# Frikallo/parakeet.cpp

Hardware: AMD Instinct MI355X
Metric: RTFx (audio-sec/wall-sec), mel+encoder+TDT decode, tdt-ctc-110m 10s@b64 (higher is better)
Workload: dtype f32; 1 GPU; tdt-ctc-110m, batch=64x10s clips per GPU, TDT greedy decode (the loops of 4 consecutive steps driven as one lock-step batch), fp32 (BASELINE configs[1]); parallelism=dp1 (utterance shards, no data-path collective), decode_group=4, decode_loop=phases, decode_overlap=1

## Files before the change

parakeet.cpp_amd/csrc/kernels/attention.hip:

```cpp
#include "attention_dev.hpp"

namespace pk {

#ifndef ATT_OCC
#define ATT_OCC 4
#endif

template <int HD, int VCH, bool SG = false, bool RAG = false, int OCC = (HD <= 64 ? ATT_OCC : 2), bool BAND = false>
__global__ __launch_bounds__(256, OCC) void relpos_attention_kernel(const float *__restrict__ qkv, int ldq, int d, int T,
                                                               const float *__restrict__ pos ,
                                                               const float *__restrict__ bias_u, const float *__restrict__ bias_v,
                                                               float scale, float *__restrict__ ctx, int PITS, int n_rb, int n_bh,
                                                               float *__restrict__ s_scratch, int ctx_bf16, int pos_row0, SeqRag rg, int left, int right) {
    static_assert(!(BAND && SG), "the band form keeps its score block in LDS");
    __builtin_amdgcn_s_setprio(3);
    constexpr int NQ4 = HD / 16;
    constexpr int VPIT = HD + 16;
    constexpr int NDV = HD / 32;
    extern __shared__ __attribute__((aligned(16))) float smem[];
    const int SPLANE = att_score_plane(PITS);
    const AttScores sc{SG ? s_scratch + (size_t)blockIdx.x * 4 * SPLANE : smem, SPLANE, PITS};
    float *VS = SG ? smem : smem + 4 * SPLANE;
    const int H = d / HD;
    AttPlace pl;
    if (!att_place<RAG, RB>(H, T, n_rb, n_bh, rg, pl)) return;
    const int h = pl.h, i0 = pl.i0;
    const int64_t row0 = pl.row0;
    T = pl.T;
    if constexpr (RAG && !BAND) pos_row0 = rg.pos_T - T;
    const int rows = (T - i0) < RB ? (T - i0) : RB;
    const AttWave w = att_wave();
    int jlo = 0, jhi = T - 1;
    if constexpr (BAND) {
        jlo = i0 - left > 0 ? i0 - left : 0;
        jhi = i0 + RB - 1 + right < T - 1 ? i0 + RB - 1 + right : T - 1;
    }
    const int W = BAND ? jhi - jlo + 1 : T;
    const int NP = BAND ? left + right + 1 : 2 * T - 1;
    const bool has_pos = BAND || pos != nullptr;
    const float *qb = qkv + row0 * ldq + h * HD;
    const float *kb = qb + d + (int64_t)jlo * ldq, *vb = qb + 2 * d + (int64_t)jlo * ldq;
    const float *pb = pos + (BAND ? (int64_t)0 : (int64_t)pos_row0 * d) + h * HD;

    float4 qx[NQ4];
    ATT_STAMP(4, 0);
    att_load_q_biased(qb, ldq, i0 + w.rt * 16, T, bias_u, h * HD, has_pos, w.l15, w.kq, qx);
    ATT_STAMP(4, 1);
    att_content_pass(sc, w, kb, ldq, W, qx, has_pos, scale);
    ATT_STAMP(4, 2);
    if (has_pos) att_load_q_biased(qb, ldq, i0 + w.rt * 16, T, bias_v, h * HD, true, w.l15, w.kq, qx);
    const int w_lo = i0 + w.rt * 16, w_hi = (w_lo + 15) < (T - 1) ? (w_lo + 15) : (T - 1);
    int wpmin = T - 1 - w_hi, wpmax = 2 * T - 2 - w_lo;
    if constexpr (BAND) {
        wpmin = jlo - w_hi + left > 0 ? jlo - w_hi + left : 0;
        wpmax = jhi - w_lo + left < NP - 1 ? jhi - w_lo + left : NP - 1;
    }
    const int npt = (has_pos && w_lo < T) ? (wpmax - wpmin) / 16 + 1 : 0;
    att_shift_pass(sc, w, pb, d, NP, wpmin, npt, BAND ? left + jlo : T - 1, i0, T, W, qx, scale);
    ATT_STAMP(4, 4);
    float4 vf[VCH * (HD / 4) / 256];
    att_v_issue<HD, VCH, 256>(vb, ldq, 0, W, vf);
    __syncthreads();
    ATT_STAMP(4, 5);
    if constexpr (BAND) {
        AttRowsBand band;
#pragma unroll
        for (int k = 0; k < RB / 4; ++k) {
            const int i = i0 + w.wave + 4 * k;
            band.clo[k] = (i - left > jlo ? i - left : jlo) - jlo;
            band.chi[k] = i < T ? (i + right < jhi ? i + right : jhi) - jlo : -1;
        }
        att_softmax(sc, w, W, ctx_bf16, band);
    } else {
        att_softmax(sc, w, W, ctx_bf16, AttRowsFull{});
    }
    ATT_STAMP(4, 6);
    att_v_commit<HD, VCH, 256>(VS, vf);
    lds_store_fence();
    __syncthreads();
    f32x4 acc[NDV];
#pragma unroll
    for (int m = 0; m < NDV; ++m) acc[m] = f32x4{0.0f, 0.0f, 0.0f, 0.0f};
    const float *sa = sc.s + w.kq * SPLANE + (w.rt * 16 + w.l15) * PITS;
    const float *vrow = VS + w.kq * VPIT + w.cp * 16 + w.l15;
    for (int c0r = 0; c0r < W; c0r += VCH) {
        const bool more = c0r + VCH < W;
        if (more) att_v_issue<HD, VCH, 256>(vb, ldq, c0r + VCH, W, vf);
        const int s_end = ((W - c0r < VCH ? W - c0r : VCH) + 3) / 4;
        att_av_steps<NDV, VPIT, SG>(sa + c0r / 4, vrow, s_end, 32, acc);
        if (more) {
            __syncthreads();
            att_v_commit<HD, VCH, 256>(VS, vf);
            lds_store_fence();
            __syncthreads();
        }
    }
#pragma unroll
    for (int m = 0; m < NDV; ++m)
#pragma unroll
        for (int r = 0; r < 4; ++r) {
            const int il = w.il_base + r;
            if (il < rows) att_store_ctx(ctx, (row0 + i0 + il) * d, h * HD + (w.cp + 2 * m) * 16 + w.l15, acc[m][r], ctx_bf16);
        }
    ATT_STAMP(4, 7);
}

static constexpr int STRIP_T = 128;

template <int HD, int VCH, int NW, int PW, bool RAG, int OCC>
__global__ __launch_bounds__(64 * NW, OCC) void relpos_attention_strip_kernel(const float *__restrict__ qkv, int ldq, int d, int T,
                                                                            const float *__restrict__ pos ,
                                                                            const float *__restrict__ bias_u, const float *__restrict__ bias_v,
                                                                            float scale, float *__restrict__ ctx, int n_rb, int n_bh, int ctx_bf16,
                                                                            int pos_row0, SeqRag rg) {
    __builtin_amdgcn_s_setprio(3);
    constexpr int NT = 64 * NW;
    constexpr int NQ4 = HD / 16, VPIT = HD + 16, NDV = HD / 16;
    constexpr int NCT = STRIP_T / 16;
    constexpr int PPIT = PW / 4 + 4, PPLANE = 16 * PPIT + 4;
    static_assert(VCH % 16 == 0 && PW % VCH == 0 && STRIP_T % PW == 0, "V chunks tile a probability piece, pieces tile the strip");
    static_assert(!RAG || NW == 2, "the units of a ragged batch are 32-row blocks");
    extern __shared__ __attribute__((aligned(16))) float smem[];
    const int H = d / HD;
    AttPlace pl;
    if (!att_place<RAG, 16 * NW>(H, T, n_rb, n_bh, rg, pl)) return;
    const int h = pl.h, i0 = pl.i0;
    const int64_t row0 = pl.row0;
    T = pl.T;
    if constexpr (RAG) pos_row0 = rg.pos_T - T;
    const int tid = threadIdx.x, lane = tid & 63, wave = tid >> 6;
    const int l15 = lane & 15, kq = lane >> 4;
    const int i_s = i0 + wave * 16;
    const bool active = i_s < T;
    const int P = 2 * T - 1;
    const int nct = (T + 15) / 16;
    const float *qb = qkv + row0 * ldq + h * HD;
    const float *kb = qb + d, *vb = qb + 2 * d;
    const float *pb = pos + (int64_t)pos_row0 * d + h * HD;
    float *VS = smem;
    float *PS = smem + VCH * VPIT + wave * 4 * PPLANE;

    float4 vf[VCH * (HD / 4) / NT];
    float4 qx[NQ4];
    ATT_STAMP(NW, 0);
    f32x4 st[NCT];
#pragma unroll
    for (int t = 0; t < NCT; ++t) st[t] = f32x4{0.0f, 0.0f, 0.0f, 0.0f};
    if (active) {
        float4 bA[NQ4], bB[NQ4];
        att_load_q_biased(qb, ldq, i_s, T, bias_u, h * HD, pos != nullptr, l15, kq, qx);
        ATT_STAMP(NW, 1);
        att_load_tile(kb, ldq, 0, T, l15, kq, bA);
#pragma unroll
        for (int t = 0; t < NCT; ++t) {
            if (t + 1 < NCT) att_load_tile(kb, ldq, (t + 1) * 16, T, l15, kq, (t & 1) ? bA : bB);
            att_mma_one(qx, (t & 1) ? bB : bA, st[t]);
            __builtin_amdgcn_sched_barrier(0);
        }
        ATT_STAMP(NW, 2);
        if (pos) {
            att_load_q_biased(qb, ldq, i_s, T, bias_v, h * HD, true, l15, kq, qx);
            const int wpmin = T - 1 - (i_s + 15);
            f32x4 pprev = f32x4{0.0f, 0.0f, 0.0f, 0.0f}, pcur;
            att_load_tile(pb, d, wpmin, P, l15, kq, bA);
#pragma unroll
            for (int u = 0; u <= NCT; ++u) {
                if (u + 1 <= NCT) att_load_tile(pb, d, wpmin + (u + 1) * 16, P, l15, kq, (u & 1) ? bA : bB);
                att_mma_one(qx, (u & 1) ? bB : bA, pcur);
                if (u >= 1) {
                    const int t = u - 1, j = t * 16 + l15;
#pragma unroll
                    for (int r = 0; r < 4; ++r) {
                        const int m = 4 * kq + r;
                        const float x = l15 >= 15 - m ? pprev[r] : pcur[r];
                        const int sl = ((lane & 48) | ((l15 - m - 1) & 15)) << 2;
                        const float a = __int_as_float(__builtin_amdgcn_ds_bpermute(sl, __float_as_int(x)));
                        st[t][r] = j < T ? (st[t][r] + a) * scale : 0.0f;
                    }
                }
                pprev = pcur;
                __builtin_amdgcn_sched_barrier(0);
            }
        } else {
#pragma unroll
            for (int t = 0; t < NCT; ++t) {
                const int j = t * 16 + l15;
#pragma unroll
                for (int r = 0; r < 4; ++r) st[t][r] = j < T ? st[t][r] * scale : 0.0f;
            }
        }
        ATT_STAMP(NW, 3);
    } else {
        ATT_STAMP(NW, 1); ATT_STAMP(NW, 2); ATT_STAMP(NW, 3);
    }
    att_v_issue<HD, VCH, NT>(vb, ldq, 0, T, vf);
    if (active) {
        float mx[4], sm[4];
#pragma unroll
        for (int r = 0; r < 4; ++r) {
            mx[r] = -__builtin_huge_valf();
#pragma unroll
            for (int t = 0; t < NCT; ++t)
                if (t * 16 + l15 < T) mx[r] = fmaxf(mx[r], st[t][r]);
        }
#pragma unroll
        for (int r = 0; r < 4; ++r) mx[r] = fmaxf(mx[r], wave_xor<8>(mx[r]));
#pragma unroll
        for (int r = 0; r < 4; ++r) mx[r] = fmaxf(mx[r], wave_xor<4>(mx[r]));
#pragma unroll
        for (int r = 0; r < 4; ++r) mx[r] = fmaxf(mx[r], wave_xor<2>(mx[r]));
#pragma unroll
        for (int r = 0; r < 4; ++r) mx[r] = fmaxf(mx[r], wave_xor<1>(mx[r]));
#pragma unroll
        for (int t = 0; t < NCT; ++t)
#pragma unroll
            for (int r = 0; r < 4; ++r) {
                const float x = st[t][r] - mx[r];
                const float e = ctx_bf16 == 1 ? __builtin_amdgcn_exp2f(x * 1.44269502162933349609375f) : dexpf_nonpos(x);
                st[t][r] = t * 16 + l15 < T ? e : 0.0f;
            }
#pragma unroll
        for (int r = 0; r < 4; ++r) {
            const float s0 = st[0][r] + st[4][r], s1 = st[1][r] + st[5][r], s2 = st[2][r] + st[6][r], s3 = st[3][r] + st[7][r];
            const float t0 = s0 + s2, t1 = s1 + s3;
            sm[r] = t0 + t1;
        }
#pragma unroll
        for (int r = 0; r < 4; ++r) sm[r] = sm[r] + wave_xor<8>(sm[r]);
#pragma unroll
        for (int r = 0; r < 4; ++r) sm[r] = sm[r] + wave_xor<4>(sm[r]);
#pragma unroll
        for (int r = 0; r < 4; ++r) sm[r] = sm[r] + wave_xor<2>(sm[r]);
#pragma unroll
        for (int r = 0; r < 4; ++r) sm[r] = sm[r] + wave_xor<1>(sm[r]);
        if (ctx_bf16 == 1) {
#pragma unroll
            for (int r = 0; r < 4; ++r) sm[r] = __builtin_amdgcn_rcpf(sm[r]);
#pragma unroll
            for (int t = 0; t < NCT; ++t)
#pragma unroll
                for (int r = 0; r < 4; ++r) st[t][r] = st[t][r] * sm[r];
        } else {
#pragma unroll
            for (int t = 0; t < NCT; ++t)
#pragma unroll
                for (int r = 0; r < 4; ++r) st[t][r] = st[t][r] / sm[r];
        }
    }
    ATT_STAMP(NW, 4);
    att_v_commit<HD, VCH, NT>(VS, vf);
    lds_store_fence();
    __syncthreads();
    ATT_STAMP(NW, 5);
    f32x4 acc[NDV];
#pragma unroll
    for (int m = 0; m < NDV; ++m) acc[m] = f32x4{0.0f, 0.0f, 0.0f, 0.0f};
    const float *vrow = VS + kq * VPIT + l15;
#pragma unroll
    for (int c = 0; c < STRIP_T / VCH; ++c) {
        const int c0r = c * VCH;
        if (c0r < T) {
            const bool more = c0r + VCH < T;
            if (more) att_v_issue<HD, VCH, NT>(vb, ldq, c0r + VCH, T, vf);
            if (active) {
                if (c0r % PW == 0) {
#pragma unroll
                    for (int tt = 0; tt < PW / 16; ++tt) {
                        const int t = c0r / 16 + tt;
                        if (t < nct) {
#pragma unroll
                            for (int r = 0; r < 4; ++r) PS[(l15 & 3) * PPLANE + (4 * kq + r) * PPIT + 4 * tt + (l15 >> 2)] = st[t][r];
                        }
                    }
                    lds_store_fence();
                }
                const int s_end = ((T - c0r < VCH ? T - c0r : VCH) + 3) / 4;
                att_av_steps<NDV, VPIT>(PS + kq * PPLANE + l15 * PPIT + (c0r % PW) / 4, vrow, s_end, 16, acc);
            }
            if (more) {
                __syncthreads();
                att_v_commit<HD, VCH, NT>(VS, vf);
                lds_store_fence();
                __syncthreads();
            }
        }
    }
    ATT_STAMP(NW, 6);
#pragma unroll
    for (int m = 0; m < NDV; ++m)
#pragma unroll
        for (int r = 0; r < 4; ++r) {
            const int i = i_s + 4 * kq + r;
            if (i < T) att_store_ctx(ctx, (row0 + i) * d, h * HD + m * 16 + l15, acc[m][r], ctx_bf16);
        }
    ATT_STAMP(NW, 7);
}

static dim3 att_grid(int n_bh, int n_rb, int n_heads, const SeqRag &rag) {
    if (rag.units.u) return dim3((unsigned)(((n_heads + 7) / 8) * 8 * (int64_t)rag.units.count));
    return dim3(((n_bh + 7) / 8) * 8 * n_rb);
}

template <int HD, int VCH, int OCC = (HD <= 64 ? ATT_OCC : 2)>
static void launch_att(const float *qkv, int B, int T, int d, int n_heads, const float *pos, const float *bias_u, const float *bias_v,
                       float *ctx, float scale_arg, hipStream_t s, float *scratch, int ctx_bf16, int pos_row0, const SeqRag &rag) {
    const float scale = scale_arg > 0.0f ? scale_arg : 1.0f / sqrtf((float)HD);
    if (rag.units.u) T = rag.T_max;
    const int pits = att_score_pitch(T);
    const int n_rb = (T + RB - 1) / RB, n_bh = B * n_heads;
    const dim3 grid = att_grid(n_bh, n_rb, n_heads, rag);
    auto go = [&](auto ragged) {
        constexpr bool RAG = decltype(ragged)::value;
        if (scratch)
            hipLaunchKernelGGL((relpos_attention_kernel<HD, VCH, true, RAG, OCC>), grid, dim3(256), (size_t)VCH * (HD + 16) * sizeof(float), s, qkv, 3 * d, d, T, pos,
                               bias_u, bias_v, scale, ctx, pits, n_rb, n_bh, scratch, ctx_bf16, pos_row0, rag, 0, 0);
        else
            att_launch_dyn_lds<relpos_attention_kernel<HD, VCH, false, RAG, OCC>>(grid, dim3(256), att_block_lds_bytes(T, HD, VCH), s, qkv, 3 * d, d, T, pos, bias_u,
                                                                                  bias_v, scale, ctx, pits, n_rb, n_bh, (float *)nullptr, ctx_bf16, pos_row0, rag, 0, 0);
    };
    if (rag.units.u) go(std::true_type{});
    else go(std::false_type{});
}

size_t relpos_attention_lds_bytes(int T, int hd) { return att_hd_supported(hd) ? att_block_lds_bytes(T, hd, att_block_vch(hd)) : 0; }
size_t relpos_attention_scratch_bytes(int B, int T, int n_heads, int hd) {
    return relpos_attention_scratch_bytes_units((T + RB - 1) / RB, T, B * n_heads, hd);
}
size_t relpos_attention_scratch_bytes_units(int64_t n_units, int T_max, int n_heads, int hd) {
    if (!att_hd_supported(hd)) return 0;
    return (size_t)((n_heads + 7) / 8) * 8 * (size_t)n_units * 4 * (size_t)att_score_plane(att_score_pitch(T_max)) * sizeof(float);
}
int relpos_attention_max_frames(int hd) {
    int T = 0;
    while (relpos_attention_lds_bytes(T + 8, hd) && relpos_attention_lds_bytes(T + 8, hd) <= 160 * 1024) T += 8;
    return T;
}

#ifndef ATT_STRIP_NW
#define ATT_STRIP_NW 4
#endif
#ifndef ATT_STRIP_VCH
#define ATT_STRIP_VCH 32
#endif
#ifndef ATT_STRIP_PW
#define ATT_STRIP_PW 64
#endif
#ifndef ATT_STRIP_DEFAULT
#define ATT_STRIP_DEFAULT 1
#endif

int relpos_attention_form(int t_longest, int hd, bool scratch, int want) {
    const bool strip_ok = !scratch && t_longest >= 1 && t_longest <= STRIP_T && (hd == 64 || hd == 32);
    if (want == ATT_FORM_STRIP) return strip_ok ? ATT_FORM_STRIP : -1;
    if (want == ATT_FORM_BLOCK) return ATT_FORM_BLOCK;
    return (ATT_STRIP_DEFAULT && strip_ok) ? ATT_FORM_STRIP : ATT_FORM_BLOCK;
}

template <int HD>
static void launch_att_strip(const float *qkv, int B, int T, int d, int n_heads, const float *pos, const float *bias_u, const float *bias_v,
                             float *ctx, float scale_arg, hipStream_t s, int ctx_bf16, int pos_row0, const SeqRag &rag) {
    const float scale = scale_arg > 0.0f ? scale_arg : 1.0f / sqrtf((float)HD);
    constexpr int VCH = ATT_STRIP_VCH, PW = ATT_STRIP_PW, NW = ATT_STRIP_NW;
    auto lds_bytes = [](int nw) { return (size_t)(VCH * (HD + 16) + nw * 4 * (16 * (PW / 4 + 4) + 4)) * sizeof(float); };
    if (rag.units.u) {
        att_launch_dyn_lds<relpos_attention_strip_kernel<HD, VCH, 2, PW, true, 4>>(att_grid(0, 0, n_heads, rag), dim3(128), lds_bytes(2), s, qkv, 3 * d, d, rag.T_max,
                                                                                   pos, bias_u, bias_v, scale, ctx, 0, 0, ctx_bf16, pos_row0, rag);
        return;
    }
    const int n_rb = (T + 16 * NW - 1) / (16 * NW), n_bh = B * n_heads;
    att_launch_dyn_lds<relpos_attention_strip_kernel<HD, VCH, NW, PW, false, 4>>(att_grid(n_bh, n_rb, n_heads, rag), dim3(64 * NW), lds_bytes(NW), s, qkv, 3 * d, d, T,
                                                                                 pos, bias_u, bias_v, scale, ctx, n_rb, n_bh, ctx_bf16, pos_row0, rag);
}

void launch_relpos_attention(const float *qkv, int B, int T, int d, int n_heads, const float *pos, const float *bias_u,
                             const float *bias_v, float *ctx, hipStream_t s, float scale, float *scratch, int ctx_bf16, int pos_row0, const SeqRag &rag,
                             int form) {
    const int hd = d / n_heads;
    if (relpos_attention_form(rag.units.u ? rag.T_max : T, hd, scratch != nullptr, form) == ATT_FORM_STRIP) {
        if (hd == 64) launch_att_strip<64>(qkv, B, T, d, n_heads, pos, bias_u, bias_v, ctx, scale, s, ctx_bf16, pos_row0, rag);
        else launch_att_strip<32>(qkv, B, T, d, n_heads, pos, bias_u, bias_v, ctx, scale, s, ctx_bf16, pos_row0, rag);
        return;
    }
    if (hd == 64) {
        const int t_lds = rag.units.u ? rag.T_max : T;
        auto occ = [&](int vch) {
            const int n = (int)((size_t)160 * 1024 / att_block_lds_bytes(t_lds, 64, vch));
            return n < ATT_OCC ? n : ATT_OCC;
        };
        if (!scratch && occ(32) > occ(64)) launch_att<64, 32>(qkv, B, T, d, n_heads, pos, bias_u, bias_v, ctx, scale, s, scratch, ctx_bf16, pos_row0, rag);
        else if (!scratch && occ(64) <= 3) launch_att<64, 64, 3>(qkv, B, T, d, n_heads, pos, bias_u, bias_v, ctx, scale, s, scratch, ctx_bf16, pos_row0, rag);
        else launch_att<64, 64>(qkv, B, T, d, n_heads, pos, bias_u, bias_v, ctx, scale, s, scratch, ctx_bf16, pos_row0, rag);
    } else if (hd == 128) launch_att<128, 32>(qkv, B, T, d, n_heads, pos, bias_u, bias_v, ctx, scale, s, scratch, ctx_bf16, pos_row0, rag);
    else if (hd == 32) launch_att<32, 64>(qkv, B, T, d, n_heads, pos, bias_u, bias_v, ctx, scale, s, scratch, ctx_bf16, pos_row0, rag);
    else if (hd == 96) launch_att<96, 64>(qkv, B, T, d, n_heads, pos, bias_u, bias_v, ctx, scale, s, scratch, ctx_bf16, pos_row0, rag);
}

template <int HD, int VCH, int OCC>
static void launch_local(const float *qkv, int B, int T, int d, int n_heads, const float *pos, const float *bias_u, const float *bias_v,
                         float *ctx, hipStream_t s, int ctx_bf16, int left, int right, int W, const SeqRag &rag) {
    const float scale = 1.0f / sqrtf((float)HD);
    const int n_rb = (T + RB - 1) / RB, n_bh = B * n_heads;
    auto go = [&](auto ragged) {
        att_launch_dyn_lds<relpos_attention_kernel<HD, VCH, false, decltype(ragged)::value, OCC, true>>(
            att_grid(n_bh, n_rb, n_heads, rag), dim3(256), att_block_lds_bytes(W, HD, VCH), s, qkv, 3 * d, d, T, pos, bias_u, bias_v, scale, ctx, att_score_pitch(W),
            n_rb, n_bh, (float *)nullptr, ctx_bf16, 0, rag, left, right);
    };
    if (rag.units.u) go(std::true_type{});
    else go(std::false_type{});
}

int relpos_local_attention_max_span(int hd) {
    if (!att_hd_supported(hd)) return -1;
    int span = -1;
    while (att_block_lds_bytes(span + 1 + RB, hd, att_block_vch(hd)) <= 160 * 1024) ++span;
    return span;
}

void launch_relpos_local_attention(const float *qkv, int B, int T, int d, int n_heads, const float *pos, const float *bias_u, const float *bias_v,
                                   float *ctx, hipStream_t s, int ctx_bf16, int left, int right, const SeqRag &rag) {
    const int hd = d / n_heads;
    const int t_lds = rag.units.u ? rag.T_max : T;
    const int W = t_lds < left + right + RB ? t_lds : left + right + RB;
    const int occ = (int)((size_t)160 * 1024 / att_block_lds_bytes(W, hd, att_block_vch(hd)));
    if (hd == 64) {
        if (occ >= 4) launch_local<64, 64, 4>(qkv, B, T, d, n_heads, pos, bias_u, bias_v, ctx, s, ctx_bf16, left, right, W, rag);
        else launch_local<64, 64, 3>(qkv, B, T, d, n_heads, pos, bias_u, bias_v, ctx, s, ctx_bf16, left, right, W, rag);
    } else if (hd == 128) launch_local<128, 32, 2>(qkv, B, T, d, n_heads, pos, bias_u, bias_v, ctx, s, ctx_bf16, left, right, W, rag);
    else if (hd == 32) launch_local<32, 64, 4>(qkv, B, T, d, n_heads, pos, bias_u, bias_v, ctx, s, ctx_bf16, left, right, W, rag);
    else if (hd == 96) launch_local<96, 64, 2>(qkv, B, T, d, n_heads, pos, bias_u, bias_v, ctx, s, ctx_bf16, left, right, W, rag);
}

}
```

parakeet.cpp_amd/csrc/kernels/attention_dev.hpp:

```cpp
#pragma once
#include "../pk_devmath.h"
#include "kernels.hpp"

namespace pk {

typedef float f32x4 __attribute__((ext_vector_type(4)));
static constexpr int RB = 32;

#ifdef ATT_TRACE
__device__ long long *att_trace;
#define ATT_STAMP(nw, i) do { if (att_trace && (threadIdx.x & 63) == 0) att_trace[((long long)blockIdx.x * (nw) + (threadIdx.x >> 6)) * 8 + (i)] = clock64(); } while (0)
#else
#define ATT_STAMP(nw, i) do { } while (0)
#endif

inline bool att_hd_supported(int hd) { return hd == 32 || hd == 64 || hd == 96 || hd == 128; }
inline int att_score_pitch(int cols) {
    int pits = (cols + 3) / 4;
    pits = (pits + 3) & ~3;
    if (((pits / 4) & 1) == 0) pits += 4;
    return pits;
}
__host__ __device__ inline int att_score_plane(int pits) { return RB * pits + 8; }
inline int att_block_vch(int hd) { return hd == 128 ? 32 : 64; }
inline size_t att_block_lds_bytes(int cols, int hd, int vch) {
    return (size_t)(4 * att_score_plane(att_score_pitch(cols)) + vch * (hd + 16)) * sizeof(float);
}

template <auto KERNEL, typename... Args>
inline void att_launch_dyn_lds(dim3 grid, dim3 block, size_t lds, hipStream_t s, Args... args) {
    static DynLdsSlots slots;
    ensure_dyn_lds(slots, reinterpret_cast<const void *>(KERNEL), lds);
    hipLaunchKernelGGL(KERNEL, grid, block, lds, s, args...);
}

__device__ __forceinline__ float f4e(const float4 &v, int e) { return e == 0 ? v.x : e == 1 ? v.y : e == 2 ? v.z : v.w; }

struct AttPlace {
    int h, i0, T;
    int64_t row0;
};
template <bool RAG, int ROWS>
__device__ __forceinline__ bool att_place(int H, int T, int n_rb, int n_bh, const SeqRag &rg, AttPlace &p) {
    const int id = blockIdx.x, xcd = id & 7, k = id >> 3;
    if constexpr (RAG) {
        p.h = (k / rg.units.count) * 8 + xcd;
        if (p.h >= H) return false;
        const RagUnit un = rg.units.u[k % rg.units.count];
        p.i0 = un.r0;
        p.T = rg.T[un.b];
        p.row0 = rg.T_off[un.b];
    } else {
        const int rbk = k % n_rb, bh = (k / n_rb) * 8 + xcd;
        if (bh >= n_bh) return false;
        p.h = bh % H;
        p.i0 = rbk * ROWS;
        p.T = T;
        p.row0 = (int64_t)(bh / H) * T;
    }
    return true;
}

template <int NQ4>
__device__ __forceinline__ void att_load_tile(const float *base, int64_t ld, int row0, int limit, int l15, int kq, float4 (&f)[NQ4]) {
    const int r = row0 + l15;
    const bool ok = r >= 0 && r < limit;
    const float *p = base + (int64_t)(ok ? r : 0) * ld + 4 * kq;
#pragma unroll
    for (int q = 0; q < NQ4; ++q) f[q] = ok ? *reinterpret_cast<const float4 *>(p + 16 * q) : make_float4(0.0f, 0.0f, 0.0f, 0.0f);
}
template <int NQ4>
__device__ __forceinline__ void att_load_q_biased(const float *qb, int ldq, int row0, int T, const float *bias, int hoff, bool biased, int l15, int kq,
                                                  float4 (&qx)[NQ4]) {
    att_load_tile(qb, ldq, row0, T, l15, kq, qx);
    if (biased) {
        const float *br = bias + hoff + kq;
#pragma unroll
        for (int f = 0; f < NQ4; ++f)
            qx[f] = make_float4(qx[f].x + br[16 * f], qx[f].y + br[16 * f + 4], qx[f].z + br[16 * f + 8], qx[f].w + br[16 * f + 12]);
    }
}
template <int NQ4>
__device__ __forceinline__ void att_mma_one(const float4 (&a)[NQ4], const float4 (&b)[NQ4], f32x4 &c) {
    c = f32x4{0.0f, 0.0f, 0.0f, 0.0f};
#pragma unroll
    for (int q = 0; q < NQ4; ++q)
#pragma unroll
        for (int e = 0; e < 4; ++e) c = __builtin_amdgcn_mfma_f32_16x16x4f32(f4e(a[q], e), f4e(b[q], e), c, 0, 0, 0);
}
template <int NQ4>
__device__ __forceinline__ void att_mma_pair(const float4 (&a)[NQ4], const float4 (&b0)[NQ4], const float4 (&b1)[NQ4], f32x4 &c0, f32x4 &c1) {
    c0 = f32x4{0.0f, 0.0f, 0.0f, 0.0f};
    c1 = f32x4{0.0f, 0.0f, 0.0f, 0.0f};
#pragma unroll
    for (int q = 0; q < NQ4; ++q)
#pragma unroll
        for (int e = 0; e < 4; ++e) {
            c0 = __builtin_amdgcn_mfma_f32_16x16x4f32(f4e(a[q], e), f4e(b0[q], e), c0, 0, 0, 0);
            c1 = __builtin_amdgcn_mfma_f32_16x16x4f32(f4e(a[q], e), f4e(b1[q], e), c1, 0, 0, 0);
        }
}

template <int HD, int VCH, int NT>
__device__ __forceinline__ void att_v_issue(const float *vb, int ldq, int row0, int limit, float4 (&vf)[VCH * (HD / 4) / NT]) {
    constexpr int KQ = HD / 4;
    static_assert((VCH * KQ) % NT == 0 && VCH % 4 == 0, "V chunk must split evenly over the workgroup's threads");
#pragma unroll
    for (int i = 0; i < VCH * KQ / NT; ++i) {
        const int e = threadIdx.x + NT * i, gr = row0 + e / KQ;
        vf[i] = make_float4(0.0f, 0.0f, 0.0f, 0.0f);
        if (gr < limit) vf[i] = *reinterpret_cast<const float4 *>(vb + (int64_t)gr * ldq + 4 * (e % KQ));
    }
}
template <int HD, int VCH, int NT>
__device__ __forceinline__ void att_v_commit(float *VS, const float4 (&vf)[VCH * (HD / 4) / NT]) {
    constexpr int KQ = HD / 4;
#pragma unroll
    for (int i = 0; i < VCH * KQ / NT; ++i) {
        const int e = threadIdx.x + NT * i;
        lds_store16(VS + (e / KQ) * (HD + 16) + 4 * (e % KQ), vf[i]);
    }
}

__device__ __forceinline__ void att_store_ctx(float *ctx, int64_t orow, int col, float v, int ctx_bf16) {
    if (ctx_bf16 == 1) reinterpret_cast<__bf16 *>(ctx)[orow + col] = (__bf16)v;
    else if (ctx_bf16 == 2) ctx[orow + sigma_col(col)] = v;
    else ctx[orow + col] = v;
}

struct AttScores {
    float *s;
    int plane, pits;
    __device__ __forceinline__ int idx(int il, int c) const { return (c & 3) * plane + il * pits + (c >> 2); }
};
struct AttWave {
    int lane, l15, kq, wave, rt, cp, il_base;
};
__device__ __forceinline__ AttWave att_wave() {
    const int tid = threadIdx.x, lane = tid & 63, wave = tid >> 6;
    return AttWave{lane, lane & 15, lane >> 4, wave, wave & 1, wave >> 1, (wave & 1) * 16 + 4 * (lane >> 4)};
}

template <int NQ4>
__device__ __forceinline__ void att_content_pass(const AttScores &sc, const AttWave &w, const float *kb, int ldq, int W, const float4 (&qx)[NQ4],
                                                 bool has_pos, float scale) {
    float *S = sc.s;
    const int Wpad4 = (W + 3) & ~3, nct = (W + 15) / 16;
    float4 bA0[NQ4], bA1[NQ4], bB0[NQ4], bB1[NQ4];
    auto load = [&](int t, float4 (&f)[NQ4]) { att_load_tile(kb, ldq, t * 16, W, w.l15, w.kq, f); };
    auto store = [&](int t, const f32x4 &a0, const f32x4 &a1) {
#pragma unroll
        for (int r = 0; r < 4; ++r) {
            const int il = w.il_base + r;
            const int c0 = t * 16 + w.l15, c1 = c0 + 32;
            if (c0 < Wpad4) S[sc.idx(il, c0)] = c0 < W ? (has_pos ? a0[r] : a0[r] * scale) : 0.0f;
            if (t + 2 < nct && c1 < Wpad4) S[sc.idx(il, c1)] = c1 < W ? (has_pos ? a1[r] : a1[r] * scale) : 0.0f;
        }
    };
    if (w.cp < nct) { load(w.cp, bA0); load(w.cp + 2, bA1); }
    for (int t = w.cp; t < nct; t += 8) {
        f32x4 a0, a1;
        if (t + 4 < nct) { load(t + 4, bB0); load(t + 6, bB1); }
        att_mma_pair(qx, bA0, bA1, a0, a1);
        store(t, a0, a1);
        if (t + 4 < nct) {
            if (t + 8 < nct) { load(t + 8, bA0); load(t + 10, bA1); }
            att_mma_pair(qx, bB0, bB1, a0, a1);
            store(t + 4, a0, a1);
        }
    }
}

template <int NQ4>
__device__ __forceinline__ void att_shift_pass(const AttScores &sc, const AttWave &w, const float *pb, int d, int NP, int wpmin, int npt, int cshift,
                                               int i0, int T, int W, const float4 (&qx)[NQ4], float scale) {
    float *S = sc.s;
    float4 bA0[NQ4], bA1[NQ4], bB0[NQ4], bB1[NQ4];
    auto load = [&](int t, float4 (&f)[NQ4]) { att_load_tile(pb, d, wpmin + t * 16, NP, w.l15, w.kq, f); };
    if (w.cp < npt) { load(w.cp, bA0); load(w.cp + 2, bA1); }
    __syncthreads();
    ATT_STAMP(4, 3);
    auto rmw = [&](int t, const f32x4 &a0, const f32x4 &a1) {
        int ad[8];
        bool ok[8];
        float v[8];
#pragma unroll
        for (int r = 0; r < 4; ++r) {
            const int il = w.il_base + r, i = i0 + il;
            const int pa = wpmin + t * 16 + w.l15, ca = pa - cshift + i;
            const int pc = pa + 32, cc = ca + 32;
            ok[r] = i < T && pa < NP && ca >= 0 && ca < W;
            ok[4 + r] = t + 2 < npt && i < T && pc < NP && cc >= 0 && cc < W;
            ad[r] = ok[r] ? sc.idx(il, ca) : 0;
            ad[4 + r] = ok[4 + r] ? sc.idx(il, cc) : 0;
        }
#pragma unroll
        for (int q = 0; q < 8; ++q) v[q] = S[ad[q]];
#pragma unroll
        for (int r = 0; r < 4; ++r) {
            if (ok[r]) S[ad[r]] = (v[r] + a0[r]) * scale;
            if (ok[4 + r]) S[ad[4 + r]] = (v[4 + r] + a1[r]) * scale;
        }
    };
    for (int t = w.cp; t < npt; t += 8) {
        f32x4 a0, a1;
        if (t + 4 < npt) { load(t + 4, bB0); load(t + 6, bB1); }
        att_mma_pair(qx, bA0, bA1, a0, a1);
        rmw(t, a0, a1);
        if (t + 4 < npt) {
            if (t + 8 < npt) { load(t + 8, bA0); load(t + 10, bA1); }
            att_mma_pair(qx, bB0, bB1, a0, a1);
            rmw(t + 4, a0, a1);
        }
    }
}

struct AttRowsFull {
    __device__ __forceinline__ bool in(int, int) const { return true; }
    __device__ __forceinline__ bool empty(int) const { return false; }
};
struct AttRowsBand {
    int clo[RB / 4], chi[RB / 4];
    __device__ __forceinline__ bool in(int k, int c) const { return c >= clo[k] && c <= chi[k]; }
    __device__ __forceinline__ bool empty(int k) const { return chi[k] < clo[k]; }
};

template <typename ROWS>
__device__ __forceinline__ void att_softmax(const AttScores &sc, const AttWave &w, int W, int ctx_bf16, const ROWS &rows) {
    float *S = sc.s;
    const int lane = w.lane, wave = w.wave;
    constexpr int NSR = RB / 4;
    float mx[NSR], sm[NSR];
#pragma unroll
    for (int k = 0; k < NSR; ++k) mx[k] = -__builtin_huge_valf();
    for (int c = lane; c < W; c += 64)
#pragma unroll
        for (int k = 0; k < NSR; ++k)
            if (rows.in(k, c)) mx[k] = fmaxf(mx[k], S[sc.idx(wave + 4 * k, c)]);
#pragma unroll
    for (int off = 32; off >= 1; off >>= 1)
#pragma unroll
        for (int k = 0; k < NSR; ++k) mx[k] = fmaxf(mx[k], __shfl_xor(mx[k], off, 64));
#pragma unroll
    for (int k = 0; k < NSR; ++k) sm[k] = 0.0f;
    for (int c = lane; c < W; c += 64) {
        float e[NSR];
#pragma unroll
        for (int k = 0; k < NSR; ++k) e[k] = S[sc.idx(wave + 4 * k, c)] - mx[k];
        if (ctx_bf16 == 1) {
#pragma unroll
            for (int k = 0; k < NSR; ++k) e[k] = __builtin_amdgcn_exp2f(e[k] * 1.44269502162933349609375f);
        } else {
#pragma unroll
            for (int k = 0; k < NSR; ++k) e[k] = dexpf_nonpos(e[k]);
        }
#pragma unroll
        for (int k = 0; k < NSR; ++k) {
            if (!rows.in(k, c)) e[k] = 0.0f;
            S[sc.idx(wave + 4 * k, c)] = e[k];
            sm[k] = sm[k] + e[k];
        }
    }
#pragma unroll
    for (int off = 32; off >= 1; off >>= 1)
#pragma unroll
        for (int k = 0; k < NSR; ++k) sm[k] = sm[k] + __shfl_xor(sm[k], off, 64);
#pragma unroll
    for (int k = 0; k < NSR; ++k) sm[k] = rows.empty(k) ? 1.0f : sm[k];
    if (ctx_bf16 == 1) {
#pragma unroll
        for (int k = 0; k < NSR; ++k) sm[k] = __builtin_amdgcn_rcpf(sm[k]);
        for (int c = lane; c < W; c += 64) {
            float e[NSR];
#pragma unroll
            for (int k = 0; k < NSR; ++k) e[k] = S[sc.idx(wave + 4 * k, c)] * sm[k];
#pragma unroll
            for (int k = 0; k < NSR; ++k) S[sc.idx(wave + 4 * k, c)] = e[k];
        }
    } else {
        for (int c = lane; c < W; c += 64) {
            float e[NSR];
#pragma unroll
            for (int k = 0; k < NSR; ++k) e[k] = S[sc.idx(wave + 4 * k, c)];
#pragma unroll
            for (int k = 0; k < NSR; ++k) e[k] = e[k] / sm[k];
#pragma unroll
            for (int k = 0; k < NSR; ++k) S[sc.idx(wave + 4 * k, c)] = e[k];
        }
    }
}

template <int NDV, int VPIT, bool GLOBAL_A = false>
__device__ __forceinline__ void att_av_steps(const float *sa, const float *vrow, int s_end, int mstride, f32x4 (&acc)[NDV]) {
    for (int s4 = 0; s4 < s_end; s4 += 4) {
        float4 a = *reinterpret_cast<const float4 *>(sa + s4);
        if constexpr (GLOBAL_A) asm volatile("" : "+v"(a.x), "+v"(a.y), "+v"(a.z), "+v"(a.w));
#pragma unroll
        for (int e = 0; e < 4; ++e) {
            if (s4 + e < s_end) {
#pragma unroll
                for (int m = 0; m < NDV; ++m)
                    acc[m] = __builtin_amdgcn_mfma_f32_16x16x4f32(f4e(a, e), vrow[(s4 + e) * 4 * VPIT + m * mstride], acc[m], 0, 0, 0);
            }
        }
    }
}

}
```

Baseline: 36600 x real-time.

## Stage K and positional rows in LDS for the strip attention kernel

Adds a staged variant of the relpos strip attention kernel. The workgroup cooperatively loads the whole K strip and the needed positional rows into LDS once, and each wave then reads its tiles from LDS instead of issuing its own redundant global loads. The relative-shift combine step is delayed by one tile to overlap with the MMAs. Defaults also change to 8 waves per block and a 64-row V chunk, with an occupancy knob. This trades more LDS per block and extra barriers, which may lower occupancy, for less global traffic.

```diff
diff --git a/parakeet.cpp_amd/csrc/kernels/attention.hip b/parakeet.cpp_amd/csrc/kernels/attention.hip
--- a/parakeet.cpp_amd/csrc/kernels/attention.hip
+++ b/parakeet.cpp_amd/csrc/kernels/attention.hip
@@ -106,8 +106,14 @@
 }
 
 static constexpr int STRIP_T = 128;
-
-template <int HD, int VCH, int NW, int PW, bool RAG, int OCC>
+#ifndef ATT_STRIP_AHEAD
+#define ATT_STRIP_AHEAD 1
+#endif
+#ifndef ATT_STRIP_LATE
+#define ATT_STRIP_LATE 1
+#endif
+
+template <int HD, int VCH, int NW, int PW, bool RAG, int OCC, bool STG = false>
 __global__ __launch_bounds__(64 * NW, OCC) void relpos_attention_strip_kernel(const float *__restrict__ qkv, int ldq, int d, int T,
                                                                             const float *__restrict__ pos ,
                                                                             const float *__restrict__ bias_u, const float *__restrict__ bias_v,
@@ -120,6 +126,7 @@
     constexpr int PPIT = PW / 4 + 4, PPLANE = 16 * PPIT + 4;
     static_assert(VCH % 16 == 0 && PW % VCH == 0 && STRIP_T % PW == 0, "V chunks tile a probability piece, pieces tile the strip");
     static_assert(!RAG || NW == 2, "the units of a ragged batch are 32-row blocks");
+    constexpr int BPIT = att_stage_pitch(HD);
     extern __shared__ __attribute__((aligned(16))) float smem[];
     const int H = d / HD;
     AttPlace pl;
@@ -139,6 +146,7 @@
     const float *pb = pos + (int64_t)pos_row0 * d + h * HD;
     float *VS = smem;
     float *PS = smem + VCH * VPIT + wave * 4 * PPLANE;
+    float *KS = smem + STRIP_T * BPIT;
 
     float4 vf[VCH * (HD / 4) / NT];
     float4 qx[NQ4];
@@ -146,29 +154,46 @@
     f32x4 st[NCT];
 #pragma unroll
     for (int t = 0; t < NCT; ++t) st[t] = f32x4{0.0f, 0.0f, 0.0f, 0.0f};
-    if (active) {
-        float4 bA[NQ4], bB[NQ4];
-        att_load_q_biased(qb, ldq, i_s, T, bias_u, h * HD, pos != nullptr, l15, kq, qx);
+    if constexpr (STG) {
+        const int wp0 = T - 1 - (i0 + 16 * NW - 1);
+        {
+            float4 kf[STRIP_T * (HD / 4) / NT], pf[STRIP_T * (HD / 4) / NT];
+            att_rows_issue<HD, STRIP_T, NT>(kb, ldq, 0, T, kf);
+            if (pos) att_rows_issue<HD, STRIP_T, NT>(pb, d, wp0, P, pf);
+            if (active) att_load_q_biased(qb, ldq, i_s, T, bias_u, h * HD, pos != nullptr, l15, kq, qx);
+            att_rows_commit<HD, STRIP_T, NT>(KS, kf);
+            if (pos) att_rows_commit<HD, STRIP_T, NT>(smem, pf);
+        }
+        lds_store_fence();
+        __syncthreads();
         ATT_STAMP(NW, 1);
-        att_load_tile(kb, ldq, 0, T, l15, kq, bA);
-#pragma unroll
-        for (int t = 0; t < NCT; ++t) {
-            if (t + 1 < NCT) att_load_tile(kb, ldq, (t + 1) * 16, T, l15, kq, (t & 1) ? bA : bB);
-            att_mma_one(qx, (t & 1) ? bB : bA, st[t]);
-            __builtin_amdgcn_sched_barrier(0);
+        constexpr int AH = ATT_STRIP_AHEAD, NB = AH + 1;
+        float4 b[NB][NQ4];
+        float4 hf[16 * NW * (HD / 4) / NT];
+        if (pos) att_rows_issue<HD, 16 * NW, NT>(pb, d, wp0 + STRIP_T, P, hf);
+        if (active) {
+            const float *kt = KS + l15 * BPIT + 4 * kq;
+#pragma unroll
+            for (int t = 0; t < AH; ++t) att_lds_tile(kt + t * 16 * BPIT, b[t]);
+#pragma unroll
+            for (int t = 0; t < NCT; ++t) {
+                if (t + AH < NCT) att_lds_tile(kt + (t + AH) * 16 * BPIT, b[(t + AH) % NB]);
+                att_mma_one(qx, b[t % NB], st[t]);
+                __builtin_amdgcn_sched_barrier(0);
+            }
         }
         ATT_STAMP(NW, 2);
         if (pos) {
-            att_load_q_biased(qb, ldq, i_s, T, bias_v, h * HD, true, l15, kq, qx);
-            const int wpmin = T - 1 - (i_s + 15);
-            f32x4 pprev = f32x4{0.0f, 0.0f, 0.0f, 0.0f}, pcur;
-            att_load_tile(pb, d, wpmin, P, l15, kq, bA);
-#pragma unroll
-            for (int u = 0; u <= NCT; ++u) {
-                if (u + 1 <= NCT) att_load_tile(pb, d, wpmin + (u + 1) * 16, P, l15, kq, (u & 1) ? bA : bB);
-                att_mma_one(qx, (u & 1) ? bB : bA, pcur);
-                if (u >= 1) {
-                    const int t = u - 1, j = t * 16 + l15;
+            if (active) att_load_q_biased(qb, ldq, i_s, T, bias_v, h * HD, true, l15, kq, qx);
+            __syncthreads();
+            att_rows_commit<HD, 16 * NW, NT>(KS, hf);
+            lds_store_fence();
+            __syncthreads();
+            if (active) {
+                const float *pt = smem + ((NW - 1 - wave) * 16 + l15) * BPIT + 4 * kq;
+                f32x4 pp[3];
+                auto combine = [&](int t, const f32x4 &pprev, const f32x4 &pcur) {
+                    const int j = t * 16 + l15;
 #pragma unroll
                     for (int r = 0; r < 4; ++r) {
                         const int m = 4 * kq + r;
@@ -177,11 +202,26 @@
                         const float a = __int_as_float(__builtin_amdgcn_ds_bpermute(sl, __float_as_int(x)));
                         st[t][r] = j < T ? (st[t][r] + a) * scale : 0.0f;
                     }
+                };
+#pragma unroll
+                for (int u = 0; u < AH; ++u) att_lds_tile(pt + u * 16 * BPIT, b[u]);
+#pragma unroll
+                for (int u = 0; u <= NCT; ++u) {
+                    if (u + AH <= NCT) att_lds_tile(pt + (u + AH) * 16 * BPIT, b[(u + AH) % NB]);
+#if ATT_STRIP_LATE
+                    if (u >= 2) combine(u - 2, pp[(u - 2) % 3], pp[(u - 1) % 3]);
+                    att_mma_one(qx, b[u % NB], pp[u % 3]);
+                    __builtin_amdgcn_sched_barrier(0);
                 }
-                pprev = pcur;
-                __builtin_amdgcn_sched_barrier(0);
-            }
-        } else {
+                combine(NCT - 1, pp[(NCT - 1) % 3], pp[NCT % 3]);
+#else
+                    att_mma_one(qx, b[u % NB], pp[u & 1]);
+                    if (u >= 1) combine(u - 1, pp[(u - 1) & 1], pp[u & 1]);
+                    __builtin_amdgcn_sched_barrier(0);
+                }
+#endif
+            }
+        } else if (active) {
 #pragma unroll
             for (int t = 0; t < NCT; ++t) {
                 const int j = t * 16 + l15;
@@ -191,7 +231,53 @@
         }
         ATT_STAMP(NW, 3);
     } else {
-        ATT_STAMP(NW, 1); ATT_STAMP(NW, 2); ATT_STAMP(NW, 3);
+        if (active) {
+            float4 bA[NQ4], bB[NQ4];
+            att_load_q_biased(qb, ldq, i_s, T, bias_u, h * HD, pos != nullptr, l15, kq, qx);
+            ATT_STAMP(NW, 1);
+            att_load_tile(kb, ldq, 0, T, l15, kq, bA);
+    #pragma unroll
+            for (int t = 0; t < NCT; ++t) {
+                if (t + 1 < NCT) att_load_tile(kb, ldq, (t + 1) * 16, T, l15, kq, (t & 1) ? bA : bB);
+                att_mma_one(qx, (t & 1) ? bB : bA, st[t]);
+                __builtin_amdgcn_sched_barrier(0);
+            }
+            ATT_STAMP(NW, 2);
+            if (pos) {
+                att_load_q_biased(qb, ldq, i_s, T, bias_v, h * HD, true, l15, kq, qx);
+                const int wpmin = T - 1 - (i_s + 15);
+                f32x4 pprev = f32x4{0.0f, 0.0f, 0.0f, 0.0f}, pcur;
+                att_load_tile(pb, d, wpmin, P, l15, kq, bA);
+    #pragma unroll
+                for (int u = 0; u <= NCT; ++u) {
+                    if (u + 1 <= NCT) att_load_tile(pb, d, wpmin + (u + 1) * 16, P, l15, kq, (u & 1) ? bA : bB);
+                    att_mma_one(qx, (u & 1) ? bB : bA, pcur);
+                    if (u >= 1) {
+                        const int t = u - 1, j = t * 16 + l15;
+    #pragma unroll
+                        for (int r = 0; r < 4; ++r) {
+                            const int m = 4 * kq + r;
+                            const float x = l15 >= 15 - m ? pprev[r] : pcur[r];
+                            const int sl = ((lane & 48) | ((l15 - m - 1) & 15)) << 2;
+                            const float a = __int_as_float(__builtin_amdgcn_ds_bpermute(sl, __float_as_int(x)));
+                            st[t][r] = j < T ? (st[t][r] + a) * scale : 0.0f;
+                        }
+                    }
+                    pprev = pcur;
+                    __builtin_amdgcn_sched_barrier(0);
+                }
+            } else {
+    #pragma unroll
+                for (int t = 0; t < NCT; ++t) {
+                    const int j = t * 16 + l15;
+    #pragma unroll
+                    for (int r = 0; r < 4; ++r) st[t][r] = j < T ? st[t][r] * scale : 0.0f;
+                }
+            }
+            ATT_STAMP(NW, 3);
+        } else {
+            ATT_STAMP(NW, 1); ATT_STAMP(NW, 2); ATT_STAMP(NW, 3);
+        }
     }
     att_v_issue<HD, VCH, NT>(vb, ldq, 0, T, vf);
     if (active) {
@@ -248,6 +334,7 @@
         }
     }
     ATT_STAMP(NW, 4);
+    if constexpr (STG) __syncthreads();
     att_v_commit<HD, VCH, NT>(VS, vf);
     lds_store_fence();
     __syncthreads();
@@ -336,14 +423,20 @@
     return T;
 }
 
+#ifndef ATT_STRIP_STAGE
+#define ATT_STRIP_STAGE 1
+#endif
 #ifndef ATT_STRIP_NW
-#define ATT_STRIP_NW 4
+#define ATT_STRIP_NW 8
 #endif
 #ifndef ATT_STRIP_VCH
-#define ATT_STRIP_VCH 32
+#define ATT_STRIP_VCH 64
 #endif
 #ifndef ATT_STRIP_PW
 #define ATT_STRIP_PW 64
+#endif
+#ifndef ATT_STRIP_OCC
+#define ATT_STRIP_OCC 4
 #endif
 #ifndef ATT_STRIP_DEFAULT
 #define ATT_STRIP_DEFAULT 1
@@ -361,15 +454,20 @@
                              float *ctx, float scale_arg, hipStream_t s, int ctx_bf16, int pos_row0, const SeqRag &rag) {
     const float scale = scale_arg > 0.0f ? scale_arg : 1.0f / sqrtf((float)HD);
     constexpr int VCH = ATT_STRIP_VCH, PW = ATT_STRIP_PW, NW = ATT_STRIP_NW;
-    auto lds_bytes = [](int nw) { return (size_t)(VCH * (HD + 16) + nw * 4 * (16 * (PW / 4 + 4) + 4)) * sizeof(float); };
+    constexpr bool STG = ATT_STRIP_STAGE != 0;
+    auto lds_bytes = [](int vch, int pw, int nw, bool stg) {
+        const size_t av = (size_t)(vch * (HD + 16) + nw * 4 * (16 * (pw / 4 + 4) + 4)), rows = stg ? (size_t)2 * STRIP_T * att_stage_pitch(HD) : 0;
+        return (av > rows ? av : rows) * sizeof(float);
+    };
     if (rag.units.u) {
-        att_launch_dyn_lds<relpos_attention_strip_kernel<HD, VCH, 2, PW, true, 4>>(att_grid(0, 0, n_heads, rag), dim3(128), lds_bytes(2), s, qkv, 3 * d, d, rag.T_max,
-                                                                                   pos, bias_u, bias_v, scale, ctx, 0, 0, ctx_bf16, pos_row0, rag);
+        att_launch_dyn_lds<relpos_attention_strip_kernel<HD, 32, 2, 64, true, 4>>(att_grid(0, 0, n_heads, rag), dim3(128), lds_bytes(32, 64, 2, false), s, qkv, 3 * d, d,
+                                                                                  rag.T_max, pos, bias_u, bias_v, scale, ctx, 0, 0, ctx_bf16, pos_row0, rag);
         return;
     }
     const int n_rb = (T + 16 * NW - 1) / (16 * NW), n_bh = B * n_heads;
-    att_launch_dyn_lds<relpos_attention_strip_kernel<HD, VCH, NW, PW, false, 4>>(att_grid(n_bh, n_rb, n_heads, rag), dim3(64 * NW), lds_bytes(NW), s, qkv, 3 * d, d, T,
-                                                                                 pos, bias_u, bias_v, scale, ctx, n_rb, n_bh, ctx_bf16, pos_row0, rag);
+    att_launch_dyn_lds<relpos_attention_strip_kernel<HD, VCH, NW, PW, false, ATT_STRIP_OCC, STG>>(att_grid(n_bh, n_rb, n_heads, rag), dim3(64 * NW), lds_bytes(VCH, PW, NW, STG),
+                                                                                                  s, qkv, 3 * d, d, T, pos, bias_u, bias_v, scale, ctx, n_rb, n_bh, ctx_bf16,
+                                                                                                  pos_row0, rag);
 }
 
 void launch_relpos_attention(const float *qkv, int B, int T, int d, int n_heads, const float *pos, const float *bias_u,
diff --git a/parakeet.cpp_amd/csrc/kernels/attention_dev.hpp b/parakeet.cpp_amd/csrc/kernels/attention_dev.hpp
--- a/parakeet.cpp_amd/csrc/kernels/attention_dev.hpp
+++ b/parakeet.cpp_amd/csrc/kernels/attention_dev.hpp
@@ -122,6 +122,33 @@
     }
 }
 
+static constexpr int att_stage_pitch(int hd) { return hd + 8; }
+template <int HD, int ROWS, int NT>
+__device__ __forceinline__ void att_rows_issue(const float *base, int64_t ld, int row0, int limit, float4 (&f)[ROWS * (HD / 4) / NT]) {
+    constexpr int KQ = HD / 4;
+    static_assert((ROWS * KQ) % NT == 0, "the rows must split evenly over the workgroup's threads");
+#pragma unroll
+    for (int i = 0; i < ROWS * KQ / NT; ++i) {
+        const int e = threadIdx.x + NT * i, gr = row0 + e / KQ;
+        f[i] = make_float4(0.0f, 0.0f, 0.0f, 0.0f);
+        if (gr >= 0 && gr < limit) f[i] = *reinterpret_cast<const float4 *>(base + (int64_t)gr * ld + 4 * (e % KQ));
+    }
+}
+template <int HD, int ROWS, int NT>
+__device__ __forceinline__ void att_rows_commit(float *dst, const float4 (&f)[ROWS * (HD / 4) / NT]) {
+    constexpr int KQ = HD / 4;
+#pragma unroll
+    for (int i = 0; i < ROWS * KQ / NT; ++i) {
+        const int e = threadIdx.x + NT * i;
+        lds_store16(dst + (e / KQ) * att_stage_pitch(HD) + 4 * (e % KQ), f[i]);
+    }
+}
+template <int NQ4>
+__device__ __forceinline__ void att_lds_tile(const float *p, float4 (&f)[NQ4]) {
+#pragma unroll
+    for (int q = 0; q < NQ4; ++q) f[q] = *reinterpret_cast<const float4 *>(p + 16 * q);
+}
+
 __device__ __forceinline__ void att_store_ctx(float *ctx, int64_t orow, int col, float v, int ctx_bf16) {
     if (ctx_bf16 == 1) reinterpret_cast<__bf16 *>(ctx)[orow + col] = (__bf16)v;
     else if (ctx_bf16 == 2) ctx[orow + sigma_col(col)] = v;
```

After: 36900 x real-time, median of 6. No clear change (+0.8%).
